# DRL-Navigation/DDRL4NAV

Measured on AMD Instinct MI355X. Metric: env-steps/sec (whole node) + PPO update ms, Pong 256 envs at 1/2/4/8 GPUs, higher is better.
Workload: dtype f32 (f16x3 MFMA planes, fp32 accumulate)

## Files before the change

### ddrl4nav_amd/csrc/wgrad2.hip

```cpp
#include <type_traits>

#include "engine2.h"

namespace ddrl {


__device__ __forceinline__ float ld_gs(const float* gs, int idx) {
  asm volatile("" : "+v"(idx));
  return gs[idx];
}

template <int I, int N, class F>
__device__ __forceinline__ void static_for(F&& f) {
  if constexpr (I < N) {
    f(std::integral_constant<int, I>{});
    static_for<I + 1, N>(f);
  }
}

struct WgradSplit {
  int pair_begin, pair_end;
  __device__ __forceinline__ void set(int n, int nsplit, int split) {
    const int npairs = (n + 1) >> 1;
    const int per = (npairs + nsplit - 1) / nsplit;
// ... 388 lines not shown
        read_b(blk + 1, b[(blk + 1) & 1]);
        if (((blk + 1) & 3) == 0) read_a(g + 1, a[(g + 1) & 1]);
      }
#pragma unroll
      for (int m = 0; m < NPROD; ++m)
#pragma unroll
        for (int i = 0; i < 2; ++i) acc[4 * i + t] = mfma_planes(a[g & 1][i][PA[m]], b[blk & 1][PB[m]], acc[4 * i + t]);
      if (j < NU) {
        if ((blk & 1) == 0) commit_unit(1 - H, j, gc);
        else fetch_unit(H, j, sf);
      }
      constexpr int PIN = 4;
      __builtin_amdgcn_sched_group_barrier(0x100, 12, 0);
#pragma unroll
      for (int k = 0; k < 2 * NPROD; ++k) {
        __builtin_amdgcn_sched_group_barrier(0x008, 1, 0);
        __builtin_amdgcn_sched_group_barrier(0x020, 2, 0);
        __builtin_amdgcn_sched_group_barrier(0x002, PIN, 0);
      }
      __builtin_amdgcn_sched_group_barrier(0x200, 2 * NPL, 0);
      __builtin_amdgcn_sched_barrier(0);
    }
  };
  if (st_begin < st_end) {
    float g0 = ld_gs(gs, st_begin);
#pragma unroll
    for (int j = 0; j < NU; ++j) fetch_unit(0, j, st_begin);
#pragma unroll
    for (int j = 0; j < NU; ++j) commit_unit(0, j, g0);
#pragma unroll
    for (int j = 0; j < NU; ++j) fetch_unit(1, j, st_begin);
    __syncthreads();
    for (int st = st_begin; st < st_end; ++st) {
      const bool more = st + 1 < st_end;
      const int sn = more ? st + 1 : st;
      const float g1 = more ? ld_gs(gs, sn) : 0.0f;
      phase(std::integral_constant<int, 0>{}, g0, sn);
      __syncthreads();
      phase(std::integral_constant<int, 1>{}, g1, sn);
      __syncthreads();
      g0 = g1;
    }
  }
  float* slab = part + ((int64_t)split * ENC_SLOTS + e) * K::SLAB;
#pragma unroll
  for (int t = 0; t < 8; ++t)
#pragma unroll
    for (int r = 0; r < 16; ++r) slab[((t / 4) * 32 + acc_row(r, hi)) * 512 + l31 * 16 + wave * 4 + t % 4] = acc[t][r] * inv;
  __syncthreads();
  float* red = (float*)ldsp;
#pragma unroll
  for (int h = 0; h < 2; ++h)
#pragma unroll
    for (int t = 0; t < K::NA; ++t)
      if (ared[h][t] >= 0) {
#pragma unroll
        for (int c = 0; c < 8; ++c) red[ared[h][t] + c] = bsum[h][t][c];
      }
  __syncthreads();
  if (tid < 64) {
    float sacc = 0.0f;
    for (int k = 0; k < 81; ++k) sacc += red[((tid >> 3) * 81 + k) * 8 + (tid & 7)];
    slab[64 * 512 + tid] = sacc;
  }
}

void launch_conv_wgrad2(const EncCall& c, float* grads, hipStream_t st) {
  const Workspace& w = *c.ws;
  const ParamLayout& L = *c.L;
  const int want = 256 / L.NE;
  const int S = c.splits->c2 < want ? c.splits->c2 : want;
  {
    ProfRange pr(c.prof, "ConvWgrad2", st);
    lds_limit_once<conv_wgrad2_pipe_kernel>((int)Wgrad2P::LDS_BYTES);
    hipLaunchKernelGGL(conv_wgrad2_pipe_kernel, dim3((unsigned)(L.NE * S)), dim3(256), Wgrad2P::LDS_BYTES, st, w.a1, w.es(A1_N), w.dz2, w.es(A2_N),
                       w.amax, w.gsc, w.es(1), w.wpart, c.n, S, L.NE);
  }
  ProfRange pr(c.prof, "reduce_partials", st);
  launch_reduce_partials(w.wpart, S, Wgrad2P::SLAB, L.NE, grads, L.enc_base[0] + L.enc.c2w, L.enc_base[1] + L.enc.c2w, st);
}

template <int NE>
struct Wgrad1B {
  static constexpr int ROWS = 32 * NE, PLANE = ROWS * 16, A_BYTES = 2 * 3 * NPL * PLANE;
  static constexpr int IMG_OFF = 2 * A_BYTES, IMG_BYTES = 2 * 4 * 16 * 192 + 64, STAGE = A_BYTES;
  static constexpr int TPE = 256 / NE, QPE = 2 * 32 * 5, NDZ_J = (QPE + TPE - 1) / TPE;
  static constexpr size_t LDS_BYTES = 2 * A_BYTES + IMG_BYTES;
};

template <int NE, bool IND = false>
__global__ __launch_bounds__(256) void conv_wgrad1_planes_kernel(const uint8_t* __restrict__ frames, const float* __restrict__ dz,
                                                                 const unsigned* __restrict__ m1, int64_t m1_es, int64_t dz_es,
                                                                 const float* __restrict__ amax, const float* __restrict__ gsc, int64_t gsc_es,
                                                                 float* __restrict__ part, int n, int nsplit, int C,
                                                                 const int32_t* __restrict__ tab, int64_t n_planes) {
  using K = Wgrad1B<NE>;
  const int fs = C * 7056;
  extern __shared__ __attribute__((aligned(16))) char ldsw[];
  const int tid = threadIdx.x, lane = tid & 63, wc = tid >> 6, l31 = lane & 31, hi = lane >> 5;
  const int split = blockIdx.y;
  WgradSplit sp;
  sp.set(n, nsplit, split);
  const int kb_begin = sp.pair_begin * 20, kb_end = sp.pair_end * 20;
  for (int i = tid; i < (int)(K::LDS_BYTES / 16); i += 256) *(f4*)(ldsw + i * 16) = zero4();
  const int ew = __builtin_amdgcn_readfirstlane(tid / K::TPE), te = tid % K::TPE;
  uint32_t dzoff[K::NDZ_J], mcol[K::NDZ_J];
  int mbit[K::NDZ_J];
  int adst[K::NDZ_J];
  unsigned dz_s1 = 0, dz_ok = 0;
  float bacc[K::NDZ_J];
#pragma unroll
  for (int j = 0; j < K::NDZ_J; ++j) {
    const int idx = te + K::TPE * j, c = min(idx, K::QPE - 1);
    const int row5 = c / 5, q4 = c % 5, smp = row5 >> 5, oc = row5 & 31, f = q4 >> 1, half = q4 & 1;
    dzoff[j] = (uint32_t)((smp * A1_N + oc * C1_P + q4 * 4) * 4);
    mcol[j] = (uint32_t)((smp * M1_N + q4 * 4) * 4);
    mbit[j] = m1_bit(oc);
    adst[j] = ((smp * 3 + f) * NPL * K::ROWS + ew * 32 + oc) * 16 + half * 8;
    dz_s1 |= (unsigned)smp << j;
    dz_ok |= (idx < K::QPE ? 1u : 0u) << j;
    bacc[j] = 0.0f;
  }
  uint32_t imoff[2];
  int bdst[2];
  unsigned im_s1 = 0, im_g1 = 0, im_ok1 = 0, im_ok2 = 0, im_tail = 0, im_ch = 0;
  int64_t imbase[2] = {0, 0};
#pragma unroll
  for (int k = 0; k < 2; ++k) {
    const int u = tid + 256 * k, uc = min(u, 383);
    const int R = uc / 6, g = uc % 6, gsel = R >> 5, smp = (R >> 4) & 1, ch = min((R >> 2) & 3, C - 1), r = R & 3;
    imoff[k] = (uint32_t)((IND ? 0 : smp * fs + ch * 7056) + (4 * gsel + r) * 84 + (g < 5 ? g * 16 : 68));
    im_ch |= (unsigned)ch << (2 * k);
    bdst[k] = K::IMG_OFF + ((smp * 4 + ch) * 16 + r) * 192 + (g < 5 ? g * 8 : 40);
    im_s1 |= (unsigned)smp << k;
    im_g1 |= (unsigned)gsel << k;
    im_ok1 |= (u < 192 ? 1u : 0u) << k;
    im_ok2 |= (u < 384 ? 1u : 0u) << k;
    im_tail |= (g == 5 ? 1u : 0u) << k;
  }
  const bool lone_group_wave = __builtin_amdgcn_readfirstlane(tid) < 192;
  const float sd = WGRAD_HEADROOM * plane_scale(amax[amax_idx(AMAX_DZ1, ew)]) / amax[amax_idx(AMAX_GMAX, ew)];
  const float* gs = gsc + ew * gsc_es;
  float gsj[K::NDZ_J];
  int aa[NE][3], bb[2][3], shamt[2], kyhi[2], kylo[2];
#pragma unroll
  for (int m = 0; m < 3; ++m) {
    const int fi = 2 * m + hi, fs = fi / 3, ff = fi % 3;
#pragma unroll
    for (int i = 0; i < NE; ++i) aa[i][m] = ((fs * 3 + ff) * NPL * K::ROWS + i * 32 + l31) * 16;
#pragma unroll
    for (int j = 0; j < 2; ++j) {
      const int c = wc * 64 + j * 32 + l31, ch = c >> 6, ky = (c >> 3) & 7, kx = c & 7;
      bb[j][m] = K::IMG_OFF + ((fs * 4 + ch) * 16) * 192 + (kx & 3) * 48 + ff * 16;
      shamt[j] = (kx >> 2) * 16;
      kyhi[j] = ky >> 2;
      kylo[j] = ky & 3;
    }
  }
  f4 dzr[K::NDZ_J];
  u4w mkr[K::NDZ_J];
  u4w imr[2] = {(u4w){0u, 0u, 0u, 0u}, (u4w){0u, 0u, 0u, 0u}};
  bool full = true, imfirst = true;
  int imam = 0;
  auto fetch = [&](int kb) __attribute__((always_inline)) {
    const int pair = kb / 20, oy = kb % 20;
    full = 2 * pair + 1 < n;
    imfirst = kb == kb_begin || oy == 0;
    const int gfirst = imfirst ? 0 : 1;
    imam = (21 * pair + oy + gfirst) & 3;
    if (imfirst) {
#pragma unroll
      for (int j = 0; j < K::NDZ_J; ++j) gsj[j] = ld_gs(gs, min(2 * pair + (int)((dz_s1 >> j) & 1u), n - 1));
      if constexpr (IND) {
#pragma unroll
        for (int k = 0; k < 2; ++k)
          imbase[k] = frame_plane_base(tab, min(2 * pair + (int)((im_s1 >> k) & 1u), n - 1), (int)((im_ch >> (2 * k)) & 3u), n_planes);
      }
    }
    const int64_t sb = ew * dz_es + (int64_t)pair * (2 * A1_N) + oy * 20;
    const char* dzb = (const char*)(dz + sb);
    const char* mb = (const char*)(m1 + ew * m1_es + (int64_t)pair * (2 * M1_N) + oy * 20);
    const char* fp = (const char*)frames + (IND ? (int64_t)0 : (int64_t)pair * (2 * fs)) + (oy + gfirst) * 336;
#pragma unroll
    for (int j = 0; j < K::NDZ_J; ++j) {
      const uint32_t o = full ? dzoff[j] : dzoff[j] - ((dz_s1 >> j) & 1u) * ((uint32_t)A1_N * 4u);
      dzr[j] = *(const f4*)(dzb + o);
      mkr[j] = *(const u4w*)(mb + (full ? mcol[j] : mcol[j] - ((dz_s1 >> j) & 1u) * ((uint32_t)M1_N * 4u)));
    }
#pragma unroll
    for (int k = 0; k < 2; ++k) {
      if (!imfirst && (k == 1 || !lone_group_wave)) continue;
      const uint32_t o = (IND || full) ? imoff[k] : imoff[k] - ((im_s1 >> k) & 1u) * (uint32_t)fs;
      const unsigned* q = (const unsigned*)(fp + (IND ? imbase[k] : (int64_t)0) + o);
      imr[k] = (u4w){q[0], q[1], q[2], q[3]};
    }
  };
  auto commit = [&](char* st) __attribute__((always_inline)) {
#pragma unroll
    for (int j = 0; j < K::NDZ_J; ++j) {
      if (j + 1 < K::NDZ_J || ((dz_ok >> j) & 1u)) {
        const f4 v = dzr[j];
        f4 g = (f4){leaky_bit(mkr[j][0], mbit[j], v.x), leaky_bit(mkr[j][1], mbit[j], v.y),
                    leaky_bit(mkr[j][2], mbit[j], v.z), leaky_bit(mkr[j][3], mbit[j], v.w)};
        if (!full && ((dz_s1 >> j) & 1u)) g = zero4();
        const float gj = gsj[j], sdj = sd * gj;
        bacc[j] += ((g.x + g.y) + (g.z + g.w)) * gj;
        unsigned pa[NPL], pb[NPL];
        split_planes(g.x, g.y, sdj, pa);
        split_planes(g.z, g.w, sdj, pb);
        char* d = st + adst[j];
#pragma unroll
        for (int p = 0; p < NPL; ++p) *(uint2*)(d + p * K::PLANE) = make_uint2(pa[p], pb[p]);
      }
    }
    const unsigned im_ok = imfirst ? im_ok2 : im_ok1;
#pragma unroll
    for (int k = 0; k < 2; ++k) {
      if ((im_ok >> k) & 1u) {
        char* d = ldsw + bdst[k] + ((imam + (int)((im_g1 >> k) & 1u)) & 3) * (4 * 192);
        if (!((im_tail >> k) & 1u)) {
          *(uint2*)(d + 0 * 48) = make_uint2(pixel_pair_sel<0, 0>(imr[k][0], imr[k][1]), pixel_pair_sel<0, 0>(imr[k][2], imr[k][3]));
          *(uint2*)(d + 1 * 48) = make_uint2(pixel_pair_sel<1, 1>(imr[k][0], imr[k][1]), pixel_pair_sel<1, 1>(imr[k][2], imr[k][3]));
          *(uint2*)(d + 2 * 48) = make_uint2(pixel_pair_sel<2, 2>(imr[k][0], imr[k][1]), pixel_pair_sel<2, 2>(imr[k][2], imr[k][3]));
          *(uint2*)(d + 3 * 48) = make_uint2(pixel_pair_sel<3, 3>(imr[k][0], imr[k][1]), pixel_pair_sel<3, 3>(imr[k][2], imr[k][3]));
        } else {
          const unsigned v = imr[k][3];
#pragma unroll
          for (int q = 0; q < 4; ++q)
            *(unsigned short*)(d + q * 48) = pixel_one((v >> (8 * q)) & 255u);
        }
      }
    }
  };
  f32x16 acc[NE][2];
#pragma unroll
  for (int i = 0; i < NE; ++i)
#pragma unroll
    for (int j = 0; j < 2; ++j)
#pragma unroll
      for (int r = 0; r < 16; ++r) acc[i][j][r] = 0.0f;
  __syncthreads();
  int kb = kb_begin;
  if (kb < kb_end) {
    fetch(kb);
    commit(ldsw);
    if (kb + 1 < kb_end) fetch(kb + 1);
  }
  __syncthreads();
  for (int buf = 0; kb < kb_end; ++kb, buf ^= 1) {
    const char* cur = ldsw + buf * K::STAGE;
    const int am = (21 * (kb / 20) + kb % 20) & 3;
    int rowoff[2];
#pragma unroll
    for (int j = 0; j < 2; ++j) rowoff[j] = ((((am + kyhi[j]) & 3) << 2) | kylo[j]) * 192;
#pragma unroll
    for (int m = 0; m < 3; ++m) {
      frag8 b[2];
#pragma unroll
      for (int j = 0; j < 2; ++j) {
        const char* q = ldsw + bb[j][m] + rowoff[j];
        const uint2 w01 = *(const uint2*)q, w23 = *(const uint2*)(q + 8);
        const unsigned w4 = *(const unsigned*)(q + 16);
        const u4w o = (u4w){__builtin_amdgcn_alignbit(w01.y, w01.x, shamt[j]), __builtin_amdgcn_alignbit(w23.x, w01.y, shamt[j]),
                            __builtin_amdgcn_alignbit(w23.y, w23.x, shamt[j]), __builtin_amdgcn_alignbit(w4, w23.y, shamt[j])};
        b[j] = __builtin_bit_cast(frag8, o);
      }
#pragma unroll
      for (int p = NPL - 1; p >= 0; --p) {
        frag8 a[NE];
#pragma unroll
        for (int i = 0; i < NE; ++i) a[i] = *(const frag8*)(cur + aa[i][m] + p * K::PLANE);
#pragma unroll
        for (int i = 0; i < NE; ++i)
#pragma unroll
          for (int j = 0; j < 2; ++j) acc[i][j] = mfma_planes(a[i], b[j], acc[i][j]);
      }
    }
    if (kb + 1 < kb_end) {
      commit(ldsw + (buf ^ 1) * K::STAGE);
      if (kb + 2 < kb_end) fetch(kb + 2);
    }
    __syncthreads();
  }
  const int ktaps = 64 * C;
  const int64_t slab_floats = slab1_floats(C);
#pragma unroll
  for (int i = 0; i < NE; ++i) {
    const float r255 = amax[amax_idx(AMAX_GMAX, i)] / (255.0f * WGRAD_HEADROOM * plane_scale(amax[amax_idx(AMAX_DZ1, i)]));
    float* slab = part + ((int64_t)split * ENC_SLOTS + i) * slab_floats;
#pragma unroll
    for (int j = 0; j < 2; ++j) {
      const int col = wc * 64 + j * 32 + l31;
      if (wc < C) {
#pragma unroll
        for (int r = 0; r < 16; ++r) slab[acc_row(r, hi) * ktaps + col] = acc[i][j][r] * r255;
      }
    }
  }
  float* red = (float*)ldsw;
#pragma unroll
  for (int j = 0; j < K::NDZ_J; ++j)
    if ((dz_ok >> j) & 1u) red[ew * K::QPE + te + K::TPE * j] = bacc[j];
  __syncthreads();
  if (tid < K::ROWS) {
    const int e = tid >> 5, oc = tid & 31;
    float sum = 0.0f;
#pragma unroll
    for (int smp = 0; smp < 2; ++smp)
#pragma unroll
      for (int q = 0; q < 5; ++q) sum += red[e * K::QPE + (smp * 32 + oc) * 5 + q];
    part[((int64_t)split * ENC_SLOTS + e) * slab_floats + 32 * ktaps + oc] = sum;
  }
}

template <int NE, bool IND>
static void launch_wgrad1_planes(const EncCall& c, int S, hipStream_t st) {
  using K = Wgrad1B<NE>;
  const Workspace& w = *c.ws;
  lds_limit_once<conv_wgrad1_planes_kernel<NE, IND>>((int)K::LDS_BYTES);
  hipLaunchKernelGGL((conv_wgrad1_planes_kernel<NE, IND>), dim3(1, S, 1), dim3(256), K::LDS_BYTES, st, c.frames, w.dz1, w.m1, w.es(M1_N),
                     w.es(A1_N), w.amax, w.gsc, w.es(1), w.wpart, c.n, S, c.L->C, c.tab, c.n_planes);
}
template <int NE>
static void launch_wgrad1(const EncCall& c, int S, hipStream_t st) {
  if (c.tab != nullptr) {
    launch_wgrad1_planes<NE, true>(c, S, st);
  } else {
    launch_wgrad1_planes<NE, false>(c, S, st);
  }
}

void launch_conv_wgrad1(const EncCall& c, float* grads, hipStream_t st) {
  const Workspace& w = *c.ws;
  const ParamLayout& L = *c.L;
  const int S = c.splits->c1;
  {
    ProfRange pr(c.prof, "ConvWgrad1", st);
    if (L.NE == 2) {
      launch_wgrad1<2>(c, S, st);
    } else {
      launch_wgrad1<1>(c, S, st);
    }
  }
  ProfRange pr(c.prof, "reduce_partials", st);
  launch_reduce_partials(w.wpart, S, slab1_floats(L.C), L.NE, grads, L.enc_base[0] + L.enc.c1w, L.enc_base[1] + L.enc.c1w, st);
}

}
```

### ddrl4nav_amd/csrc/conv2.hip

```cpp
#include "engine2.h"

namespace ddrl {


using u4v = __attribute__((ext_vector_type(4))) unsigned;

constexpr int F1_PITCH = 168;
template <int NE>
struct Fwd1B {
  static constexpr int ROWS = 32 * NE, A_BYTES = 4 * NPL * 2 * ROWS * 16, PITCH = F1_PITCH, IMG_BYTES = 64 * PITCH;
  static constexpr int STAGE_BYTES = A_BYTES + IMG_BYTES, AQ = A_BYTES / 16, NAJ = AQ / 256;
  static constexpr size_t LDS_BYTES = 2 * STAGE_BYTES;
};

template <int NE, bool IND = false>
__global__ __launch_bounds__(256) void conv_fwd1_planes_kernel(const uint8_t* __restrict__ frames, const unsigned short* __restrict__ wp1b,
                                                               float* __restrict__ amax, const float* __restrict__ params, int64_t bias_off0,
                                                               int64_t bias_off1, float* __restrict__ out, int64_t out_es, int n,
                                                               unsigned* __restrict__ m1, int64_t m1_es, int C,
                                                               const int32_t* __restrict__ tab, int64_t n_planes) {
  using K = Fwd1B<NE>;
  extern __shared__ __attribute__((aligned(16))) char ldsb[];
  const int tid = threadIdx.x, lane = tid & 63, wc = tid >> 6, l31 = lane & 31, hi = lane >> 5;
  const int c0 = blockIdx.x * 256, ctot = n * C1_P, clast = min(c0 + 255, ctot - 1);
// ... 565 lines not shown
  fetch(0);
  commit();
  fetch(1);
  __syncthreads();
  for (int kb = 0; kb < NKB; ++kb) {
#pragma unroll
    for (int kg = 0; kg < 5; ++kg) {
      frag8 a[NPL][2], b[NPL][K::TN];
#pragma unroll
      for (int p = 0; p < NPL; ++p) {
#pragma unroll
        for (int i = 0; i < 2; ++i) a[p][i] = *(const frag8*)(ldsc3 + aA[i] + (kg * NPL + p) * 2048);
#pragma unroll
        for (int j = 0; j < K::TN; ++j) b[p][j] = *(const frag8*)(ldsc3 + bB[j] + tapoff[kg] + p * K::IMG_PLANE);
      }
#pragma unroll
      for (int t = 0; t < NPROD; ++t)
#pragma unroll
        for (int i = 0; i < 2; ++i)
#pragma unroll
          for (int j = 0; j < K::TN; ++j) acc[i][j] = mfma_planes(a[PA[t]][i], b[PB[t]][j], acc[i][j]);
    }
    __syncthreads();
    if (kb + 1 < NKB) {
      commit();
      if (kb + 2 < NKB) fetch(kb + 2);
    }
    __syncthreads();
  }
  const float* bias = (const float*)(ldsc3 + K::BIAS_OFF);
  float big = 0.0f;
#pragma unroll
  for (int j = 0; j < K::TN; ++j) {
    const int c = wc * (32 * K::TN) + j * 32 + l31;
    const int s = c / 49, pix = c % 49;
    if (c >= K::SPT * 49 || b0 + s >= n) continue;
    float* base = out + e * out_es + (int64_t)b0 * FLAT;
    const uint32_t lb = (uint32_t)((s * A3_N + pix + hi * (4 * C3_P)) * 4);
    unsigned bits = 0u;
#pragma unroll
    for (int i = 0; i < 2; ++i)
#pragma unroll
      for (int r = 0; r < 16; ++r) {
        const int oc = i * 32 + acc_row(r, hi);
        const float y = leaky_f(__builtin_fmaf(acc[i][j][r], inv, bias[oc]));
        st1_so(base + (i * 32 + acc_row(r, 0)) * C3_P, lb, y);
        big = fmaxf(big, fabsf(y));
        bits = __builtin_amdgcn_alignbit(bits, (unsigned)__builtin_elementwise_sub_sat((int)__float_as_uint(y), 1), 31);
      }
    if (m3 != nullptr) m3[(e * (out_es / A3_N) + b0 + s) * M3_N + pix * 2 + hi] = (bits >> 16) | (bits << 16);
  }
  amax_update(big, amax + amax_idx(AMAX_A3, e));
}
static void launch_fwd3_planes(const EncCall& c, bool acting, hipStream_t st) {
  using K = Fwd3B;
  const Workspace& w = *c.ws;
  const ParamLayout& L = *c.L;
  lds_limit_once<conv_fwd3_planes_kernel>((int)K::LDS_BYTES);
  hipLaunchKernelGGL(conv_fwd3_planes_kernel, dim3((unsigned)((c.n + K::SPT - 1) / K::SPT), 1, (unsigned)L.NE), dim3(256), K::LDS_BYTES, st, w.a2,
                     w.es(A2_N), w.wp3b, w.amax, c.params, L.enc_base[0] + L.enc.c3b, L.enc_base[L.NE - 1] + L.enc.c3b, w.a3, w.es(A3_N),
                     c.n, acting ? (unsigned*)nullptr : w.m3);
}


void launch_conv_forward(const EncCall& c, bool acting, hipStream_t st) {
  {
    ProfRange pr(c.prof, acting ? "ConvFwd1.act" : "ConvFwd1", st);
    if (c.L->NE == 2) {
      launch_fwd1<2>(c, acting, st);
    } else {
      launch_fwd1<1>(c, acting, st);
    }
  }
  {
    ProfRange pr(c.prof, acting ? "ConvFwd2.act" : "ConvFwd2", st);
    launch_fwd2_planes(c, acting, st);
  }
  {
    ProfRange pr(c.prof, acting ? "ConvFwd3.act" : "ConvFwd3", st);
    launch_fwd3_planes(c, acting, st);
  }
}

struct Dgrad3B {
  static constexpr int THREADS = 256, TN = 2, SPT = ((THREADS / 64) * 32 * TN) / 81;
  static constexpr int KOC = 16, NKB = 64 / KOC, PIXB = 2 * KOC;
  static constexpr int IMG_PLANE = SPT * 121 * PIXB;
  static constexpr int W_OFF = NPL * IMG_PLANE, W_BYTES = 9 * NPL * 64 * 32;
  static constexpr int NIU = SPT * 49, NIJ = (NIU + THREADS - 1) / THREADS;
  static constexpr int NWQ = W_BYTES / 16, NWJ = (NWQ + THREADS - 1) / THREADS;
  static constexpr size_t LDS_BYTES = W_OFF + W_BYTES;
};

__global__ __launch_bounds__(Dgrad3B::THREADS) __attribute__((amdgpu_waves_per_eu(2, 2))) void conv_dgrad3_planes_kernel(
    const float* __restrict__ dz3, int64_t dz_es, const unsigned short* __restrict__ wd3b, float* __restrict__ amax, const unsigned* __restrict__ m2,
    float* __restrict__ out, int64_t out_es, int n) {
  using K = Dgrad3B;
  extern __shared__ __attribute__((aligned(16))) char ldsd3[];
  const int tid = threadIdx.x, lane = tid & 63, wc = tid >> 6, l31 = lane & 31, hi = lane >> 5;
  const int e = blockIdx.z, b0 = blockIdx.x * K::SPT;
  const float sa = plane_scale(amax[amax_idx(AMAX_DZ3, e)]), inv = 1.0f / (sa * plane_scale(amax[amax_idx(AMAX_W3, e)]));
  for (int i = tid; i < K::W_OFF / 16; i += K::THREADS) *(f4*)(ldsd3 + i * 16) = zero4();
  const float* isrc[K::NIJ];
  int idst[K::NIJ];
#pragma unroll
  for (int j = 0; j < K::NIJ; ++j) {
    const int u = min(tid + K::THREADS * j, K::NIU - 1);
    const int s = u / 49, px = u % 49;
    isrc[j] = dz3 + e * dz_es + (int64_t)min(b0 + s, n - 1) * FLAT + px;
    idst[j] = (s * 121 + (px / 7 + 2) * 11 + px % 7 + 2) * K::PIXB;
  }
  const unsigned short* wsrc = wd3b + (int64_t)e * (K::NKB * 9 * NPL * 64 * 16) + tid * 8;
  int aA[2], bB[K::TN];
#pragma unroll
  for (int i = 0; i < 2; ++i) aA[i] = K::W_OFF + (i * 32 + l31) * 32 + hi * 16;
#pragma unroll
  for (int j = 0; j < K::TN; ++j) {
    int c = wc * (32 * K::TN) + j * 32 + l31;
    if (c >= K::SPT * 81) c = 0;
    const int s = c / 81, pix = c % 81;
    bB[j] = (s * 121 + (pix / 9 + 2) * 11 + pix % 9 + 2) * K::PIXB + hi * 16;
  }
  float ir[K::NIJ][K::KOC];
  f4 wr[K::NWJ];
  auto fetch = [&](int kb) {
#pragma unroll
    for (int j = 0; j < K::NIJ; ++j)
#pragma unroll
      for (int c = 0; c < K::KOC; ++c) ir[j][c] = isrc[j][(kb * K::KOC + c) * C3_P];
#pragma unroll
    for (int j = 0; j < K::NWJ; ++j)
      if (j + 1 < K::NWJ || tid + K::THREADS * j < K::NWQ) wr[j] = *(const f4*)(wsrc + kb * (9 * NPL * 1024) + j * (K::THREADS * 8));
  };
  auto commit = [&]() {
#pragma unroll
    for (int j = 0; j < K::NIJ; ++j) {
      if (j + 1 < K::NIJ || tid + K::THREADS * j < K::NIU) {
        unsigned pl[K::KOC / 2][NPL];
#pragma unroll
        for (int c = 0; c < K::KOC / 2; ++c) split_planes(ir[j][2 * c], ir[j][2 * c + 1], sa, pl[c]);
        char* d = ldsd3 + idst[j];
#pragma unroll
        for (int p = 0; p < NPL; ++p) {
          *(u4v*)(d + p * K::IMG_PLANE) = (u4v){pl[0][p], pl[1][p], pl[2][p], pl[3][p]};
          *(u4v*)(d + p * K::IMG_PLANE + 16) = (u4v){pl[4][p], pl[5][p], pl[6][p], pl[7][p]};
        }
      }
    }
#pragma unroll
    for (int j = 0; j < K::NWJ; ++j)
      if (j + 1 < K::NWJ || tid + K::THREADS * j < K::NWQ) *(f4*)(ldsd3 + K::W_OFF + (tid + K::THREADS * j) * 16) = wr[j];
  };
  f32x16 acc[2][K::TN];
#pragma unroll
  for (int i = 0; i < 2; ++i)
#pragma unroll
    for (int j = 0; j < K::TN; ++j)
#pragma unroll
      for (int r = 0; r < 16; ++r) acc[i][j][r] = 0.0f;
  fetch(0);
  __syncthreads();
  commit();
  fetch(1);
  __syncthreads();
  for (int kb = 0; kb < K::NKB; ++kb) {
#pragma unroll
    for (int t = 0; t < 9; ++t) {
      constexpr int ROW11 = 11;
      const int toff = ((t / 3) * ROW11 + t % 3) * K::PIXB;
      frag8 af[NPL][2], bfr[NPL][K::TN];
#pragma unroll
      for (int p = 0; p < NPL; ++p) {
#pragma unroll
        for (int i = 0; i < 2; ++i) af[p][i] = *(const frag8*)(ldsd3 + aA[i] + (t * NPL + p) * 2048);
#pragma unroll
        for (int j = 0; j < K::TN; ++j) bfr[p][j] = *(const frag8*)(ldsd3 + bB[j] - toff + p * K::IMG_PLANE);
      }
#pragma unroll
      for (int m = 0; m < NPROD; ++m)
#pragma unroll
        for (int i = 0; i < 2; ++i)
#pragma unroll
          for (int j = 0; j < K::TN; ++j) acc[i][j] = mfma_planes(af[PA[m]][i], bfr[PB[m]][j], acc[i][j]);
    }
    __syncthreads();
    if (kb + 1 < K::NKB) {
      commit();
      if (kb + 2 < K::NKB) fetch(kb + 2);
    }
    __syncthreads();
  }
  float big = 0.0f;
#pragma unroll
  for (int j = 0; j < K::TN; ++j) {
    const int c = wc * (32 * K::TN) + j * 32 + l31;
    const int s = c / 81, pix = c % 81;
    if (c >= K::SPT * 81 || b0 + s >= n) continue;
    const int64_t off = (int64_t)(b0 + s) * A2_N + pix + hi * (4 * C2_P);
    float* op = out + e * out_es + off;
    const unsigned mw = m2[(e * (out_es / A2_N) + b0 + s) * M2_N + pix * 2 + hi];
#pragma unroll
    for (int i = 0; i < 2; ++i)
#pragma unroll
      for (int r = 0; r < 16; ++r) {
        const float g = leaky_bit(mw, 16 * i + 15 - r, acc[i][j][r] * inv);
        op[(i * 32 + acc_row(r, 0)) * C2_P] = g;
        big = fmaxf(big, fabsf(g));
      }
  }
  amax_update(big, amax + amax_idx(AMAX_DZ2, e));
}
static void launch_dgrad3_planes(const EncCall& c, hipStream_t st) {
  using K = Dgrad3B;
  const Workspace& w = *c.ws;
  lds_limit_once<conv_dgrad3_planes_kernel>((int)K::LDS_BYTES);
  hipLaunchKernelGGL(conv_dgrad3_planes_kernel, dim3((unsigned)((c.n + K::SPT - 1) / K::SPT), 1, (unsigned)c.L->NE), dim3(K::THREADS), K::LDS_BYTES, st,
                     w.dz3, w.es(A3_N), w.wd3b, w.amax, w.m2, w.dz2, w.es(A2_N), c.n);
}

void launch_conv_dgrad3(const EncCall& c, hipStream_t st) {
  ProfRange pr(c.prof, "ConvDgrad3", st);
  launch_dgrad3_planes(c, st);
}

struct Dgrad2Both {
  static constexpr int SPT = 5, THREADS = 512, TN = 2;
  static constexpr int IMG_PLANE = SPT * 121 * 16;
  static constexpr int W_HALF = 2 * NPL * 64 * 32;
  static constexpr int W_OFF = NPL * IMG_PLANE, W_BYTES = 2 * W_HALF;
  static constexpr int NIU = SPT * 81;
  static constexpr int NWQ = W_BYTES / 16, NWJ = NWQ / THREADS;
  static constexpr size_t LDS_BYTES = W_OFF + W_BYTES;
};

__global__ __launch_bounds__(512) __attribute__((amdgpu_waves_per_eu(2, 2))) void conv_dgrad2_both_kernel(
    const float* __restrict__ dz2, int64_t dz_es, const unsigned short* __restrict__ wd2b, float* __restrict__ amax, float* __restrict__ out,
    int64_t out_es, int n) {
  using K = Dgrad2Both;
  extern __shared__ __attribute__((aligned(16))) char ldsd2[];
  const int tid = threadIdx.x, lane = tid & 63, wc = tid >> 6, l31 = lane & 31, hi = lane >> 5;
  const int e = blockIdx.y, b0 = blockIdx.x * K::SPT;
  const float sa = plane_scale(amax[amax_idx(AMAX_DZ2, e)]), inv = 1.0f / (sa * plane_scale(amax[amax_idx(AMAX_W2, e)]));
  for (int i = tid; i < K::W_OFF / 16; i += K::THREADS) *(f4*)(ldsd2 + i * 16) = zero4();
  const int u = min(tid, K::NIU - 1);
  const float* isrc = dz2 + e * dz_es + (int64_t)min(b0 + u / C2_P, n - 1) * A2_N + u % C2_P;
  const int idst = ((u / 81) * 121 + ((u % 81) / 9 + 1) * 11 + (u % 81) % 9 + 1) * 16;
  const unsigned short* wsrc[K::NWJ];
#pragma unroll
  for (int j = 0; j < K::NWJ; ++j) {
    const int q = tid + K::THREADS * j, par = q / (K::W_HALF / 16), qh = q % (K::W_HALF / 16);
    wsrc[j] = wd2b + (int64_t)(e * 2 + par) * (8 * 2 * NPL * 64 * 16) + qh * 8;
  }
  int aA[4], bB[K::TN];
#pragma unroll
  for (int i = 0; i < 4; ++i) aA[i] = K::W_OFF + (i >> 1) * K::W_HALF + ((i & 1) * 32 + l31) * 32 + hi * 16;
#pragma unroll
  for (int j = 0; j < K::TN; ++j) {
    int c = wc * (32 * K::TN) + j * 32 + l31;
    if (c >= K::SPT * 100) c = 0;
    const int s = c / 100, pq = c % 100;
    bB[j] = (s * 121 + (pq / 10 + 1) * 11 + (pq % 10 + 1) - hi) * 16;
  }
  float ir[8];
  f4 wr[K::NWJ];
  auto fetch = [&](int kb) {
#pragma unroll
    for (int c = 0; c < 8; ++c) ir[c] = isrc[(kb * 8 + c) * C2_P];
#pragma unroll
    for (int j = 0; j < K::NWJ; ++j) wr[j] = *(const f4*)(wsrc[j] + kb * (2 * NPL * 1024));
  };
  auto commit = [&]() {
    if (tid < K::NIU) {
      unsigned pl[4][NPL];
#pragma unroll
      for (int c = 0; c < 4; ++c) split_planes(ir[2 * c], ir[2 * c + 1], sa, pl[c]);
      char* d = ldsd2 + idst;
#pragma unroll
      for (int p = 0; p < NPL; ++p) *(u4v*)(d + p * K::IMG_PLANE) = (u4v){pl[0][p], pl[1][p], pl[2][p], pl[3][p]};
    }
#pragma unroll
    for (int j = 0; j < K::NWJ; ++j) *(f4*)(ldsd2 + K::W_OFF + (tid + K::THREADS * j) * 16) = wr[j];
  };
  f32x16 acc[4][K::TN];
#pragma unroll
  for (int i = 0; i < 4; ++i)
#pragma unroll
    for (int j = 0; j < K::TN; ++j)
#pragma unroll
      for (int r = 0; r < 16; ++r) acc[i][j][r] = 0.0f;
  constexpr int NKB = 8;
  fetch(0);
// ... 59 lines not shown
```

Baseline: 256,700.

## Process two output rows per wgrad1 k-block with a six-group image ring

The conv1 weight-gradient kernel now covers two output rows per k-block instead of one. It stages ten dz fragments per stage and keeps a six-group image ring buffer rather than a four-group one, and the MFMA loop runs five fragment steps per block with a remapped B-operand gather. The aim is to halve the number of k-block iterations and barriers and to reuse the loaded image rows across more MFMAs. In exchange it uses more LDS (asserted at or under 80KB so two workgroups still fit per CU) and more complex indexing that could raise register pressure.

New measurement: 258,200, median of 6. No clear change (+0.6%).

```diff
diff --git a/ddrl4nav_amd/csrc/wgrad2.hip b/ddrl4nav_amd/csrc/wgrad2.hip
--- a/ddrl4nav_amd/csrc/wgrad2.hip
+++ b/ddrl4nav_amd/csrc/wgrad2.hip
@@ -494,10 +494,14 @@
 
 template <int NE>
 struct Wgrad1B {
-  static constexpr int ROWS = 32 * NE, PLANE = ROWS * 16, A_BYTES = 2 * 3 * NPL * PLANE;
-  static constexpr int IMG_OFF = 2 * A_BYTES, IMG_BYTES = 2 * 4 * 16 * 192 + 64, STAGE = A_BYTES;
-  static constexpr int TPE = 256 / NE, QPE = 2 * 32 * 5, NDZ_J = (QPE + TPE - 1) / TPE;
+  static constexpr int ROWS = 32 * NE, PLANE = ROWS * 16, NFRAG = 10, A_BYTES = NFRAG * NPL * PLANE;
+  static constexpr int NRING = 6, RING_ROWS = 4 * NRING, IMG_SMP = 4 * RING_ROWS * 192;
+  static constexpr int IMG_OFF = 2 * A_BYTES, IMG_BYTES = 2 * IMG_SMP, STAGE = A_BYTES;
+  static constexpr int KB_PAIR = 10, GROUPS_PAIR = 21;
+  static constexpr int TPE = 256 / NE, QPE = 2 * 32 * 10, NDZ_J = (QPE + TPE - 1) / TPE;
+  static constexpr int NIM = 3;
   static constexpr size_t LDS_BYTES = 2 * A_BYTES + IMG_BYTES;
+  static_assert(LDS_BYTES <= 80 * 1024 && LDS_BYTES % 16 == 0, "two workgroups per CU");
 };
 
 template <int NE, bool IND = false>
@@ -513,7 +517,7 @@
   const int split = blockIdx.y;
   WgradSplit sp;
   sp.set(n, nsplit, split);
-  const int kb_begin = sp.pair_begin * 20, kb_end = sp.pair_end * 20;
+  const int kb_begin = sp.pair_begin * K::KB_PAIR, kb_end = sp.pair_end * K::KB_PAIR;
   for (int i = tid; i < (int)(K::LDS_BYTES / 16); i += 256) *(f4*)(ldsw + i * 16) = zero4();
   const int ew = __builtin_amdgcn_readfirstlane(tid / K::TPE), te = tid % K::TPE;
   uint32_t dzoff[K::NDZ_J], mcol[K::NDZ_J];
@@ -524,75 +528,72 @@
 #pragma unroll
   for (int j = 0; j < K::NDZ_J; ++j) {
     const int idx = te + K::TPE * j, c = min(idx, K::QPE - 1);
-    const int row5 = c / 5, q4 = c % 5, smp = row5 >> 5, oc = row5 & 31, f = q4 >> 1, half = q4 & 1;
-    dzoff[j] = (uint32_t)((smp * A1_N + oc * C1_P + q4 * 4) * 4);
-    mcol[j] = (uint32_t)((smp * M1_N + q4 * 4) * 4);
+    const int row10 = c / 10, q10 = c % 10, smp = row10 >> 5, oc = row10 & 31, row = q10 / 5, q4 = q10 % 5;
+    const int F = 5 * row + (q4 == 4 ? 2 : 3 * smp + (q4 >> 1)), half = q4 == 4 ? smp : (q4 & 1);
+    dzoff[j] = (uint32_t)((smp * A1_N + oc * C1_P + q10 * 4) * 4);
+    mcol[j] = (uint32_t)((smp * M1_N + q10 * 4) * 4);
     mbit[j] = m1_bit(oc);
-    adst[j] = ((smp * 3 + f) * NPL * K::ROWS + ew * 32 + oc) * 16 + half * 8;
+    adst[j] = (F * NPL * K::ROWS + ew * 32 + oc) * 16 + half * 8;
     dz_s1 |= (unsigned)smp << j;
     dz_ok |= (idx < K::QPE ? 1u : 0u) << j;
     bacc[j] = 0.0f;
   }
-  uint32_t imoff[2];
-  int bdst[2];
-  unsigned im_s1 = 0, im_g1 = 0, im_ok1 = 0, im_ok2 = 0, im_tail = 0, im_ch = 0;
-  int64_t imbase[2] = {0, 0};
-#pragma unroll
-  for (int k = 0; k < 2; ++k) {
-    const int u = tid + 256 * k, uc = min(u, 383);
+  uint32_t imoff[K::NIM];
+  int bdst[K::NIM];
+  unsigned im_s1 = 0, im_gv = 0, im_ok2 = 0, im_ok3 = 0, im_tail = 0, im_ch = 0;
+  int64_t imbase[K::NIM] = {0, 0, 0};
+#pragma unroll
+  for (int k = 0; k < K::NIM; ++k) {
+    const int u = tid + 256 * k, uc = min(u, 575);
     const int R = uc / 6, g = uc % 6, gsel = R >> 5, smp = (R >> 4) & 1, ch = min((R >> 2) & 3, C - 1), r = R & 3;
     imoff[k] = (uint32_t)((IND ? 0 : smp * fs + ch * 7056) + (4 * gsel + r) * 84 + (g < 5 ? g * 16 : 68));
     im_ch |= (unsigned)ch << (2 * k);
-    bdst[k] = K::IMG_OFF + ((smp * 4 + ch) * 16 + r) * 192 + (g < 5 ? g * 8 : 40);
+    bdst[k] = K::IMG_OFF + ((smp * 4 + ch) * K::RING_ROWS + r) * 192 + (g < 5 ? g * 8 : 40);
     im_s1 |= (unsigned)smp << k;
-    im_g1 |= (unsigned)gsel << k;
-    im_ok1 |= (u < 192 ? 1u : 0u) << k;
+    im_gv |= (unsigned)gsel << (2 * k);
     im_ok2 |= (u < 384 ? 1u : 0u) << k;
+    im_ok3 |= (u < 576 ? 1u : 0u) << k;
     im_tail |= (g == 5 ? 1u : 0u) << k;
   }
-  const bool lone_group_wave = __builtin_amdgcn_readfirstlane(tid) < 192;
+  const unsigned im_g = __builtin_amdgcn_readfirstlane(im_gv);
+  const int wv = __builtin_amdgcn_readfirstlane(tid) >> 6;
   const float sd = WGRAD_HEADROOM * plane_scale(amax[amax_idx(AMAX_DZ1, ew)]) / amax[amax_idx(AMAX_GMAX, ew)];
   const float* gs = gsc + ew * gsc_es;
   float gsj[K::NDZ_J];
-  int aa[NE][3], bb[2][3], shamt[2], kyhi[2], kylo[2];
-#pragma unroll
-  for (int m = 0; m < 3; ++m) {
-    const int fi = 2 * m + hi, fs = fi / 3, ff = fi % 3;
-#pragma unroll
-    for (int i = 0; i < NE; ++i) aa[i][m] = ((fs * 3 + ff) * NPL * K::ROWS + i * 32 + l31) * 16;
-#pragma unroll
-    for (int j = 0; j < 2; ++j) {
-      const int c = wc * 64 + j * 32 + l31, ch = c >> 6, ky = (c >> 3) & 7, kx = c & 7;
-      bb[j][m] = K::IMG_OFF + ((fs * 4 + ch) * 16) * 192 + (kx & 3) * 48 + ff * 16;
-      shamt[j] = (kx >> 2) * 16;
-      kyhi[j] = ky >> 2;
-      kylo[j] = ky & 3;
-    }
-  }
+  int aa[NE];
+#pragma unroll
+  for (int i = 0; i < NE; ++i) aa[i] = (hi * NPL * K::ROWS + i * 32 + l31) * 16;
+  const int kx = l31 & 7, kylo = l31 >> 3, shamt = (kx >> 2) * 16;
+  const int cb = K::IMG_OFF + wc * K::RING_ROWS * 192 + (kx & 3) * 48;
+  const int bo[3] = {cb + hi * 16, cb + (hi ? 0 : K::IMG_SMP + 16), cb + K::IMG_SMP + hi * 16};
+  const int blo[2] = {cb + (hi ? K::IMG_SMP : 32), cb + (hi ? 32 : 16)};
+  const int bup[2] = {cb + K::IMG_SMP + (hi ? 8 : 32), cb + (hi ? K::IMG_SMP + 32 : 24)};
   f4 dzr[K::NDZ_J];
   u4w mkr[K::NDZ_J];
-  u4w imr[2] = {(u4w){0u, 0u, 0u, 0u}, (u4w){0u, 0u, 0u, 0u}};
+  u4w imr[K::NIM];
+#pragma unroll
+  for (int k = 0; k < K::NIM; ++k) imr[k] = (u4w){0u, 0u, 0u, 0u};
   bool full = true, imfirst = true;
   int imam = 0;
   auto fetch = [&](int kb) __attribute__((always_inline)) {
-    const int pair = kb / 20, oy = kb % 20;
+    const int pair = kb / K::KB_PAIR, b = kb % K::KB_PAIR;
     full = 2 * pair + 1 < n;
-    imfirst = kb == kb_begin || oy == 0;
+    imfirst = kb == kb_begin || b == 0;
     const int gfirst = imfirst ? 0 : 1;
-    imam = (21 * pair + oy + gfirst) & 3;
+    imam = (K::GROUPS_PAIR * pair + 2 * b + gfirst) % K::NRING;
     if (imfirst) {
 #pragma unroll
       for (int j = 0; j < K::NDZ_J; ++j) gsj[j] = ld_gs(gs, min(2 * pair + (int)((dz_s1 >> j) & 1u), n - 1));
       if constexpr (IND) {
 #pragma unroll
-        for (int k = 0; k < 2; ++k)
+        for (int k = 0; k < K::NIM; ++k)
           imbase[k] = frame_plane_base(tab, min(2 * pair + (int)((im_s1 >> k) & 1u), n - 1), (int)((im_ch >> (2 * k)) & 3u), n_planes);
       }
     }
-    const int64_t sb = ew * dz_es + (int64_t)pair * (2 * A1_N) + oy * 20;
+    const int64_t sb = ew * dz_es + (int64_t)pair * (2 * A1_N) + b * 40;
     const char* dzb = (const char*)(dz + sb);
-    const char* mb = (const char*)(m1 + ew * m1_es + (int64_t)pair * (2 * M1_N) + oy * 20);
-    const char* fp = (const char*)frames + (IND ? (int64_t)0 : (int64_t)pair * (2 * fs)) + (oy + gfirst) * 336;
+    const char* mb = (const char*)(m1 + ew * m1_es + (int64_t)pair * (2 * M1_N) + b * 40);
+    const char* fp = (const char*)frames + (IND ? (int64_t)0 : (int64_t)pair * (2 * fs)) + (2 * b + gfirst) * 336;
 #pragma unroll
     for (int j = 0; j < K::NDZ_J; ++j) {
       const uint32_t o = full ? dzoff[j] : dzoff[j] - ((dz_s1 >> j) & 1u) * ((uint32_t)A1_N * 4u);
@@ -600,8 +601,8 @@
       mkr[j] = *(const u4w*)(mb + (full ? mcol[j] : mcol[j] - ((dz_s1 >> j) & 1u) * ((uint32_t)M1_N * 4u)));
     }
 #pragma unroll
-    for (int k = 0; k < 2; ++k) {
-      if (!imfirst && (k == 1 || !lone_group_wave)) continue;
+    for (int k = 0; k < K::NIM; ++k) {
+      if (imfirst ? (k == 2 && wv > 0) : (k == 2 || (k == 1 && wv > 1))) continue;
       const uint32_t o = (IND || full) ? imoff[k] : imoff[k] - ((im_s1 >> k) & 1u) * (uint32_t)fs;
       const unsigned* q = (const unsigned*)(fp + (IND ? imbase[k] : (int64_t)0) + o);
       imr[k] = (u4w){q[0], q[1], q[2], q[3]};
@@ -625,11 +626,12 @@
         for (int p = 0; p < NPL; ++p) *(uint2*)(d + p * K::PLANE) = make_uint2(pa[p], pb[p]);
       }
     }
-    const unsigned im_ok = imfirst ? im_ok2 : im_ok1;
-#pragma unroll
-    for (int k = 0; k < 2; ++k) {
+    const unsigned im_ok = imfirst ? im_ok3 : im_ok2;
+#pragma unroll
+    for (int k = 0; k < K::NIM; ++k) {
       if ((im_ok >> k) & 1u) {
-        char* d = ldsw + bdst[k] + ((imam + (int)((im_g1 >> k) & 1u)) & 3) * (4 * 192);
+        const int rg = imam + (int)((im_g >> (2 * k)) & 3u);
+        char* d = ldsw + bdst[k] + (rg >= K::NRING ? rg - K::NRING : rg) * (4 * 192);
         if (!((im_tail >> k) & 1u)) {
           *(uint2*)(d + 0 * 48) = make_uint2(pixel_pair_sel<0, 0>(imr[k][0], imr[k][1]), pixel_pair_sel<0, 0>(imr[k][2], imr[k][3]));
           *(uint2*)(d + 1 * 48) = make_uint2(pixel_pair_sel<1, 1>(imr[k][0], imr[k][1]), pixel_pair_sel<1, 1>(imr[k][2], imr[k][3]));
@@ -661,27 +663,43 @@
   __syncthreads();
   for (int buf = 0; kb < kb_end; ++kb, buf ^= 1) {
     const char* cur = ldsw + buf * K::STAGE;
-    const int am = (21 * (kb / 20) + kb % 20) & 3;
-    int rowoff[2];
-#pragma unroll
-    for (int j = 0; j < 2; ++j) rowoff[j] = ((((am + kyhi[j]) & 3) << 2) | kylo[j]) * 192;
-#pragma unroll
-    for (int m = 0; m < 3; ++m) {
+    const int am = (K::GROUPS_PAIR * (kb / K::KB_PAIR) + 2 * (kb % K::KB_PAIR)) % K::NRING;
+    int ro[3], rmid[2];
+#pragma unroll
+    for (int i = 0; i < 3; ++i) ro[i] = ((am + i >= K::NRING ? am + i - K::NRING : am + i) * 4 + kylo) * 192;
+#pragma unroll
+    for (int j = 0; j < 2; ++j) {
+      const int g = am + j + hi;
+      rmid[j] = ((g >= K::NRING ? g - K::NRING : g) * 4 + kylo) * 192;
+    }
+#pragma unroll
+    for (int m = 0; m < 5; ++m) {
       frag8 b[2];
 #pragma unroll
       for (int j = 0; j < 2; ++j) {
-        const char* q = ldsw + bb[j][m] + rowoff[j];
-        const uint2 w01 = *(const uint2*)q, w23 = *(const uint2*)(q + 8);
-        const unsigned w4 = *(const unsigned*)(q + 16);
-        const u4w o = (u4w){__builtin_amdgcn_alignbit(w01.y, w01.x, shamt[j]), __builtin_amdgcn_alignbit(w23.x, w01.y, shamt[j]),
-                            __builtin_amdgcn_alignbit(w23.y, w23.x, shamt[j]), __builtin_amdgcn_alignbit(w4, w23.y, shamt[j])};
+        const int rowoff = m < 2 ? ro[j] : m > 2 ? ro[j + 1] : rmid[j];
+        u4w o;
+        if (m & 1) {
+          const char* ql = ldsw + blo[m >> 1] + rowoff;
+          const char* qu = ldsw + bup[m >> 1] + rowoff;
+          const uint2 l01 = *(const uint2*)ql, u01 = *(const uint2*)qu;
+          const unsigned l2 = *(const unsigned*)(ql + 8), u2 = *(const unsigned*)(qu + 8);
+          o = (u4w){__builtin_amdgcn_alignbit(l01.y, l01.x, shamt), __builtin_amdgcn_alignbit(l2, l01.y, shamt),
+                    __builtin_amdgcn_alignbit(u01.y, u01.x, shamt), __builtin_amdgcn_alignbit(u2, u01.y, shamt)};
+        } else {
+          const char* q = ldsw + bo[m >> 1] + rowoff;
+          const uint2 w01 = *(const uint2*)q, w23 = *(const uint2*)(q + 8);
+          const unsigned w4 = *(const unsigned*)(q + 16);
+          o = (u4w){__builtin_amdgcn_alignbit(w01.y, w01.x, shamt), __builtin_amdgcn_alignbit(w23.x, w01.y, shamt),
+                    __builtin_amdgcn_alignbit(w23.y, w23.x, shamt), __builtin_amdgcn_alignbit(w4, w23.y, shamt)};
+        }
         b[j] = __builtin_bit_cast(frag8, o);
       }
 #pragma unroll
       for (int p = NPL - 1; p >= 0; --p) {
         frag8 a[NE];
 #pragma unroll
-        for (int i = 0; i < NE; ++i) a[i] = *(const frag8*)(cur + aa[i][m] + p * K::PLANE);
+        for (int i = 0; i < NE; ++i) a[i] = *(const frag8*)(cur + aa[i] + (2 * m * NPL + p) * K::PLANE);
 #pragma unroll
         for (int i = 0; i < NE; ++i)
 #pragma unroll
@@ -720,7 +738,7 @@
 #pragma unroll
     for (int smp = 0; smp < 2; ++smp)
 #pragma unroll
-      for (int q = 0; q < 5; ++q) sum += red[e * K::QPE + (smp * 32 + oc) * 5 + q];
+      for (int q = 0; q < 10; ++q) sum += red[e * K::QPE + (smp * 32 + oc) * 10 + q];
     part[((int64_t)split * ENC_SLOTS + e) * slab_floats + 32 * ktaps + oc] = sum;
   }
 }
```

## Reorder dgrad3 columns by row and skip zero-border taps with balanced wave roles

Applied to the files above, without the earlier changes.

Column tiles in the conv3 data-gradient kernel now follow a row-major (row, sample, x) order, so a 32-column tile spans only a few output rows. Taps that would read only the zero border are then dropped at compile time, leaving 60 of 72 tile-tap products per row tile, and a static assignment spreads the accumulator tiles over the four waves so each issues the same number of MFMAs. The output is first staged through LDS and written back as 16-byte vector stores instead of scattered scalar stores. SPT changes from the old formula to 3, and the per-wave templated code paths make the kernel larger and may raise register pressure.

Result: faster. 244,500 before, 247,900 after (median of 6 runs) (+1.4%).

```diff
diff --git a/ddrl4nav_amd/csrc/conv2.hip b/ddrl4nav_amd/csrc/conv2.hip
--- a/ddrl4nav_amd/csrc/conv2.hip
+++ b/ddrl4nav_amd/csrc/conv2.hip
@@ -671,22 +671,117 @@
   }
 }
 
+struct Dgrad3Rows {
+  static constexpr int SPT = 3, NCOL = SPT * 81, NT = 8, ROWW = SPT * 9;
+  static constexpr int col_y(int c) { return c / ROWW; }
+  static constexpr int col_s(int c) { return c % ROWW / 9; }
+  static constexpr int col_x(int c) { return c % 9; }
+  static constexpr int tile_y0(int t) { return col_y(32 * t); }
+  static constexpr int tile_y1(int t) { return col_y(32 * t + 31 < NCOL ? 32 * t + 31 : NCOL - 1); }
+  static constexpr bool tile_has_tap(int t, int tap) { return tap / 3 <= tile_y1(t) && tap / 3 + 6 >= tile_y0(t); }
+  static constexpr int tile_taps(int t) {
+    int m = 0;
+    for (int tap = 0; tap < 9; ++tap) m |= (int)tile_has_tap(t, tap) << tap;
+    return m;
+  }
+  static constexpr int WT = 3, NU = 4;
+  static constexpr int WAVE_TILE[4][WT] = {{0, 1, -1}, {5, 6, -1}, {2, 3, 7}, {4, 3, 7}};
+  static constexpr int UNIT_I[4][NU] = {{0, 1, 0, 1}, {0, 1, 0, 1}, {0, 1, 0, 0}, {0, 1, 1, 1}};
+  static constexpr int UNIT_J[4][NU] = {{0, 0, 1, 1}, {0, 0, 1, 1}, {0, 0, 1, 2}, {0, 0, 1, 2}};
+  static constexpr int unit_tile(int w, int u) { return WAVE_TILE[w][UNIT_J[w][u]]; }
+  static constexpr int popcount9(int m) {
+    int c = 0;
+    for (int b = 0; b < 9; ++b) c += m >> b & 1;
+    return c;
+  }
+
+  static constexpr bool tap_feeds_tile(int t, int tap) {
+    for (int c = 32 * t; c < 32 * t + 32 && c < NCOL; ++c) {
+      const int sy = col_y(c) - tap / 3, sx = col_x(c) - tap % 3;
+      if (sy >= 0 && sy <= 6 && sx >= 0 && sx <= 6) return true;
+    }
+    return false;
+  }
+  static constexpr bool masks_are_exact() {
+    for (int t = 0; t < NT; ++t)
+      for (int tap = 0; tap < 9; ++tap)
+        if (tap_feeds_tile(t, tap) != tile_has_tap(t, tap)) return false;
+    return true;
+  }
+  static constexpr bool columns_are_a_permutation() {
+    bool seen[NCOL] = {};
+    for (int c = 0; c < NCOL; ++c) {
+      const int k = col_s(c) * 81 + col_y(c) * 9 + col_x(c);
+      if (col_s(c) >= SPT || col_y(c) >= 9 || seen[k]) return false;
+      seen[k] = true;
+    }
+    return true;
+  }
+  static constexpr int owners(int i, int t) {
+    int n = 0;
+    for (int w = 0; w < 4; ++w)
+      for (int u = 0; u < NU; ++u) n += UNIT_I[w][u] == i && UNIT_J[w][u] < WT && unit_tile(w, u) == t;
+    return n;
+  }
+  static constexpr bool every_unit_has_one_owner() {
+    for (int i = 0; i < 2; ++i)
+      for (int t = 0; t < NT; ++t)
+        if (owners(i, t) != 1) return false;
+    return true;
+  }
+  static constexpr int wave_unit_taps(int w) {
+    int n = 0;
+    for (int u = 0; u < NU; ++u) n += popcount9(tile_taps(unit_tile(w, u)));
+    return n;
+  }
+  static constexpr int row_tile_taps() {
+    int n = 0;
+    for (int t = 0; t < NT; ++t) n += popcount9(tile_taps(t));
+    return n;
+  }
+};
+static_assert(Dgrad3Rows::NT * 32 >= Dgrad3Rows::NCOL && (Dgrad3Rows::NT - 1) * 32 < Dgrad3Rows::NCOL, "8 column tiles of 32");
+static_assert(Dgrad3Rows::columns_are_a_permutation(), "every (sample, pixel) is one column");
+static_assert(Dgrad3Rows::masks_are_exact(), "a skipped (tile, tap) reads only the zero border, an issued one reads a dz3 pixel");
+static_assert(Dgrad3Rows::every_unit_has_one_owner(), "each of the 16 accumulator tiles belongs to exactly one wave (four each)");
+static_assert(Dgrad3Rows::row_tile_taps() == 60, "60 of 72 (column tile, tap) products per row tile");
+static_assert(Dgrad3Rows::wave_unit_taps(0) == 30 && Dgrad3Rows::wave_unit_taps(1) == 30 && Dgrad3Rows::wave_unit_taps(2) == 30 &&
+                  Dgrad3Rows::wave_unit_taps(3) == 30, "the waves are level: 30 unit-taps = 90 MFMAs per k-block each");
+
+template <int V>
+struct RoleC {
+  static constexpr int value = V;
+};
+template <class F>
+__device__ __forceinline__ void by_wave_role(int w, F&& f) {
+  switch (w) {
+    case 0: f(RoleC<0>{}); break;
+    case 1: f(RoleC<1>{}); break;
+    case 2: f(RoleC<2>{}); break;
+    default: f(RoleC<3>{}); break;
+  }
+}
+
 struct Dgrad3B {
-  static constexpr int THREADS = 256, TN = 2, SPT = ((THREADS / 64) * 32 * TN) / 81;
+  using R = Dgrad3Rows;
+  static constexpr int THREADS = 256, SPT = R::SPT;
   static constexpr int KOC = 16, NKB = 64 / KOC, PIXB = 2 * KOC;
   static constexpr int IMG_PLANE = SPT * 121 * PIXB;
   static constexpr int W_OFF = NPL * IMG_PLANE, W_BYTES = 9 * NPL * 64 * 32;
   static constexpr int NIU = SPT * 49, NIJ = (NIU + THREADS - 1) / THREADS;
   static constexpr int NWQ = W_BYTES / 16, NWJ = (NWQ + THREADS - 1) / THREADS;
   static constexpr size_t LDS_BYTES = W_OFF + W_BYTES;
+  static constexpr int OSS = 32 * C2_P + 16, OQS = 32 * C2_P / 4, NOJ = (SPT * OQS + THREADS - 1) / THREADS;
+  static_assert(SPT * OSS * 4 <= (int)LDS_BYTES && (32 * C2_P) % 4 == 0 && OSS % 4 == 0 && A2_N % 4 == 0, "the staged half fits, 16-byte rows");
 };
 
 __global__ __launch_bounds__(Dgrad3B::THREADS) __attribute__((amdgpu_waves_per_eu(2, 2))) void conv_dgrad3_planes_kernel(
     const float* __restrict__ dz3, int64_t dz_es, const unsigned short* __restrict__ wd3b, float* __restrict__ amax, const unsigned* __restrict__ m2,
     float* __restrict__ out, int64_t out_es, int n) {
   using K = Dgrad3B;
+  using R = K::R;
   extern __shared__ __attribute__((aligned(16))) char ldsd3[];
-  const int tid = threadIdx.x, lane = tid & 63, wc = tid >> 6, l31 = lane & 31, hi = lane >> 5;
+  const int tid = threadIdx.x, lane = tid & 63, wc = __builtin_amdgcn_readfirstlane(tid >> 6), l31 = lane & 31, hi = lane >> 5;
   const int e = blockIdx.z, b0 = blockIdx.x * K::SPT;
   const float sa = plane_scale(amax[amax_idx(AMAX_DZ3, e)]), inv = 1.0f / (sa * plane_scale(amax[amax_idx(AMAX_W3, e)]));
   for (int i = tid; i < K::W_OFF / 16; i += K::THREADS) *(f4*)(ldsd3 + i * 16) = zero4();
@@ -700,16 +795,18 @@
     idst[j] = (s * 121 + (px / 7 + 2) * 11 + px % 7 + 2) * K::PIXB;
   }
   const unsigned short* wsrc = wd3b + (int64_t)e * (K::NKB * 9 * NPL * 64 * 16) + tid * 8;
-  int aA[2], bB[K::TN];
+  int aA[2], bB[R::WT];
 #pragma unroll
   for (int i = 0; i < 2; ++i) aA[i] = K::W_OFF + (i * 32 + l31) * 32 + hi * 16;
-#pragma unroll
-  for (int j = 0; j < K::TN; ++j) {
-    int c = wc * (32 * K::TN) + j * 32 + l31;
-    if (c >= K::SPT * 81) c = 0;
-    const int s = c / 81, pix = c % 81;
-    bB[j] = (s * 121 + (pix / 9 + 2) * 11 + pix % 9 + 2) * K::PIXB + hi * 16;
-  }
+  by_wave_role(wc, [&](auto role) {
+    constexpr int W = decltype(role)::value;
+#pragma unroll
+    for (int j = 0; j < R::WT; ++j) {
+      int c = R::WAVE_TILE[W][j] * 32 + l31;
+      if (R::WAVE_TILE[W][j] < 0 || c >= R::NCOL) c = 0;
+      bB[j] = (R::col_s(c) * 121 + R::col_y(c) * 11 + R::col_x(c)) * K::PIXB + hi * 16;
+    }
+  });
   float ir[K::NIJ][K::KOC];
   f4 wr[K::NWJ];
   auto fetch = [&](int kb) {
@@ -740,62 +837,87 @@
     for (int j = 0; j < K::NWJ; ++j)
       if (j + 1 < K::NWJ || tid + K::THREADS * j < K::NWQ) *(f4*)(ldsd3 + K::W_OFF + (tid + K::THREADS * j) * 16) = wr[j];
   };
-  f32x16 acc[2][K::TN];
-#pragma unroll
-  for (int i = 0; i < 2; ++i)
-#pragma unroll
-    for (int j = 0; j < K::TN; ++j)
-#pragma unroll
-      for (int r = 0; r < 16; ++r) acc[i][j][r] = 0.0f;
+  f32x16 acc[R::NU];
+#pragma unroll
+  for (int u = 0; u < R::NU; ++u)
+#pragma unroll
+    for (int r = 0; r < 16; ++r) acc[u][r] = 0.0f;
+  auto mma = [&](auto role) {
+    constexpr int W = decltype(role)::value;
+#pragma unroll
+    for (int t = 0; t < 9; ++t) {
+      constexpr int ROW11 = 11;
+      const int toff = ((2 - t / 3) * ROW11 + 2 - t % 3) * K::PIXB;
+      frag8 af[NPL][2], bfr[NPL][R::WT];
+#pragma unroll
+      for (int p = 0; p < NPL; ++p) {
+#pragma unroll
+        for (int i = 0; i < 2; ++i) af[p][i] = *(const frag8*)(ldsd3 + aA[i] + (t * NPL + p) * 2048);
+#pragma unroll
+        for (int j = 0; j < R::WT; ++j)
+          if (R::WAVE_TILE[W][j] >= 0 && R::tile_has_tap(R::WAVE_TILE[W][j], t)) bfr[p][j] = *(const frag8*)(ldsd3 + bB[j] + toff + p * K::IMG_PLANE);
+      }
+#pragma unroll
+      for (int m = 0; m < NPROD; ++m)
+#pragma unroll
+        for (int u = 0; u < R::NU; ++u)
+          if (R::tile_has_tap(R::unit_tile(W, u), t)) acc[u] = mfma_planes(af[PA[m]][R::UNIT_I[W][u]], bfr[PB[m]][R::UNIT_J[W][u]], acc[u]);
+    }
+  };
   fetch(0);
   __syncthreads();
   commit();
   fetch(1);
   __syncthreads();
-  for (int kb = 0; kb < K::NKB; ++kb) {
-#pragma unroll
-    for (int t = 0; t < 9; ++t) {
-      constexpr int ROW11 = 11;
-      const int toff = ((t / 3) * ROW11 + t % 3) * K::PIXB;
-      frag8 af[NPL][2], bfr[NPL][K::TN];
-#pragma unroll
-      for (int p = 0; p < NPL; ++p) {
-#pragma unroll
-        for (int i = 0; i < 2; ++i) af[p][i] = *(const frag8*)(ldsd3 + aA[i] + (t * NPL + p) * 2048);
-#pragma unroll
-        for (int j = 0; j < K::TN; ++j) bfr[p][j] = *(const frag8*)(ldsd3 + bB[j] - toff + p * K::IMG_PLANE);
-      }
-#pragma unroll
-      for (int m = 0; m < NPROD; ++m)
-#pragma unroll
-        for (int i = 0; i < 2; ++i)
-#pragma unroll
-          for (int j = 0; j < K::TN; ++j) acc[i][j] = mfma_planes(af[PA[m]][i], bfr[PB[m]][j], acc[i][j]);
-    }
+  by_wave_role(wc, [&](auto role) {
+    for (int kb = 0; kb < K::NKB; ++kb) {
+      mma(role);
+      __syncthreads();
+      if (kb + 1 < K::NKB) {
+        commit();
+        if (kb + 2 < K::NKB) fetch(kb + 2);
+      }
+      __syncthreads();
+    }
+  });
+  float big = 0.0f;
+  float* ob = (float*)ldsd3;
+  unsigned mw[R::WT];
+  int ocol[R::WT];
+  by_wave_role(wc, [&](auto role) {
+    constexpr int W = decltype(role)::value;
+#pragma unroll
+    for (int j = 0; j < R::WT; ++j) {
+      const int c = R::WAVE_TILE[W][j] * 32 + l31;
+      const int s = R::col_s(c), pix = R::col_y(c) * 9 + R::col_x(c);
+      const bool live = R::WAVE_TILE[W][j] >= 0 && c < R::NCOL && b0 + s < n;
+      ocol[j] = live ? s * K::OSS + hi * (4 * C2_P) + pix : -1;
+      mw[j] = live ? m2[(e * (out_es / A2_N) + b0 + s) * M2_N + pix * 2 + hi] : 0u;
+    }
+  });
+#pragma unroll
+  for (int i = 0; i < 2; ++i) {
+    if (i) __syncthreads();
+    by_wave_role(wc, [&](auto role) {
+      constexpr int W = decltype(role)::value;
+#pragma unroll
+      for (int u = 0; u < R::NU; ++u) {
+        const int j = R::UNIT_J[W][u];
+        if (R::UNIT_I[W][u] != i || ocol[j] < 0) continue;
+#pragma unroll
+        for (int r = 0; r < 16; ++r) {
+          const float g = leaky_bit(mw[j], 16 * i + 15 - r, acc[u][r] * inv);
+          ob[ocol[j] + acc_row(r, 0) * C2_P] = g;
+          big = fmaxf(big, fabsf(g));
+        }
+      }
+    });
     __syncthreads();
-    if (kb + 1 < K::NKB) {
-      commit();
-      if (kb + 2 < K::NKB) fetch(kb + 2);
-    }
-    __syncthreads();
-  }
-  float big = 0.0f;
-#pragma unroll
-  for (int j = 0; j < K::TN; ++j) {
-    const int c = wc * (32 * K::TN) + j * 32 + l31;
-    const int s = c / 81, pix = c % 81;
-    if (c >= K::SPT * 81 || b0 + s >= n) continue;
-    const int64_t off = (int64_t)(b0 + s) * A2_N + pix + hi * (4 * C2_P);
-    float* op = out + e * out_es + off;
-    const unsigned mw = m2[(e * (out_es / A2_N) + b0 + s) * M2_N + pix * 2 + hi];
-#pragma unroll
-    for (int i = 0; i < 2; ++i)
-#pragma unroll
-      for (int r = 0; r < 16; ++r) {
-        const float g = leaky_bit(mw, 16 * i + 15 - r, acc[i][j][r] * inv);
-        op[(i * 32 + acc_row(r, 0)) * C2_P] = g;
-        big = fmaxf(big, fabsf(g));
-      }
+#pragma unroll
+    for (int k = 0; k < K::NOJ; ++k) {
+      const int q = tid + K::THREADS * k, s = q / K::OQS, w4 = q % K::OQS * 4;
+      if (q < K::SPT * K::OQS && b0 + s < n) *(f4*)(out + e * out_es + (int64_t)(b0 + s) * A2_N + i * (32 * C2_P) + w4) = *(const f4*)(ob + s * K::OSS + w4);
+    }
   }
   amax_update(big, amax + amax_idx(AMAX_DZ2, e));
 }
```
